# stevengiacalone/triceratops

Hardware: AMD Instinct MI355X
Metric: light-curve-point x sample evals/sec (higher is better)
Workload: dtype f64

## Files before the change

include/trx_debug.h:

```cpp
#ifndef TRX_DEBUG_H
#define TRX_DEBUG_H

#include "trx.h"

#ifdef __cplusplus
extern "C" {
#endif

int trx_set_rows_per_wave(int rows);
int trx_set_cell_packing_below(int n_time);
int trx_debug_batch_plan(long rows, int rows_per_wave, int taper, long* positions, int* rows_min);

int trx_set_supersample_tiers(int on);
int trx_set_stencil(int on);
int trx_set_skip_excluded(int on);
int trx_set_debug_node_counts(int on);
int trx_set_kepler_stepping(int on);

int trx_set_bounded_evaluation(int mode);
int trx_set_debug_bounded_lnl(int on);
int trx_set_debug_poison(int on);
int trx_set_debug_bug(int on);
int trx_set_probe_rows(int rows);
int trx_set_star_chain(int on);
int trx_debug_chain_counts(long* chains, long* calls_in_chains, long* posterior_calls_in_chains, int reset);

int trx_debug_capture_buffers(long* live, long* idle);

#ifdef __cplusplus
}
#endif
#endif
```

triceratops_amd/_lib.py:

```python
import ctypes
import os
import threading

import numpy as np
import torch

_HERE = os.path.dirname(os.path.abspath(__file__))
LIB_PATH = os.environ.get("TRX_LIB") or os.path.join(_HERE, "libtrx.so")
TESTING_LIB_PATH = os.environ.get("TRX_TESTING_LIB") or os.path.join(_HERE, "libtrx_testing.so")

MODEL_TP, MODEL_EB, MODEL_EB_TWIN, MODEL_RAW = 0, 1, 2, 3
FLAG_COMPANION_IS_HOST, FLAG_SCALAR_K, FLAG_FP32_MODEL, FLAG_EVALUATE_EXCLUDED = 1, 2, 4, 8
FLAG_ALL_SUBEXPOSURES, FLAG_NO_STENCIL, FLAG_COUNT_EVALUATIONS, FLAG_FULL_EVALUATION = 16, 32, 64, 128
FLAG_WEIGHT_MOMENTS = 256
N_PARAM = {MODEL_TP: 10, MODEL_EB: 11, MODEL_EB_TWIN: 11, MODEL_RAW: 9}
ERR_NTOTAL = 4

ABI_SYMBOLS = (
    "trx_lnl_batch", "trx_lnl_batch_weighted", "trx_flux_grid", "trx_chi2_grid", "trx_chi2_grid_weighted",
    "trx_chi2_grid_offset", "trx_chi2_grid_baseline", "trx_workspace_bytes",
    "trx_log_mean_exp", "trx_lnz_scenario", "trx_lnz_from_halfchi2", "trx_lnz_moments_from_halfchi2",
    "trx_posterior_from_halfchi2", "trx_grid_quantiles",
    "trx_lnl_batch_host", "trx_flux_grid_host",
    "trx_log_mean_exp_host", "trx_skipped_rows", "trx_pruned_rows",
    "trx_draw_scenario", "trx_draw_args_size", "trx_scenario_evidence", "trx_scenario_enqueue", "trx_star_enqueue",
    "trx_scenario_args_size", "trx_release_scratch", "trx_version", "trx_last_error", "trx_device_count",
)
DEBUG_SYMBOLS = (
    "trx_set_rows_per_wave", "trx_set_cell_packing_below", "trx_debug_batch_plan", "trx_set_supersample_tiers",
    "trx_set_stencil", "trx_set_skip_excluded", "trx_set_debug_node_counts", "trx_set_kepler_stepping",
    "trx_set_bounded_evaluation", "trx_set_debug_bounded_lnl", "trx_set_debug_poison", "trx_set_debug_bug",
    "trx_set_probe_rows", "trx_set_star_chain", "trx_debug_capture_buffers", "trx_debug_chain_counts",
)


class TrxError(RuntimeError):
    pass


EXTRA_FLAGS = 0
CELL_PACKING_BELOW = 320
STATS = {"rows": 0, "cells": 0, "launches": 0, "native_calls": 0}
_stats_lock = threading.Lock()


def count_launch(rows, n_time):
    with _stats_lock:
        STATS["rows"] += rows
        STATS["cells"] += rows * n_time
        STATS["launches"] += 1
TRACE = None
TRACE_SAMPLE_ROWS = 128


def reset_stats():
# ... 89 lines not shown
    L.trx_posterior_from_halfchi2.argtypes = [_vp, _vp, c_long, c_double, c_int, ctypes.c_ulonglong, _vp, _vp, _vp,
                                              c_size_t, _vp]
    L.trx_grid_quantiles.restype = c_int
    L.trx_grid_quantiles.argtypes = [_vp, c_long, c_int, _vp, _vp, c_long, _vp, c_int, _vp, _vp]
    L.trx_lnl_batch_host.restype = c_int
    L.trx_lnl_batch_host.argtypes = [c_int, c_int, _vp, _vp, c_int, c_double, _vp, c_long,
                                     c_double, c_int, _vp]
    L.trx_flux_grid_host.restype = c_int
    L.trx_flux_grid_host.argtypes = [c_int, c_int, _vp, c_int, _vp, c_long, c_double, c_int, _vp, _vp]
    L.trx_log_mean_exp_host.restype = c_int
    L.trx_log_mean_exp_host.argtypes = [_vp, c_long, c_long, _vp]
    L.trx_skipped_rows.restype = c_int
    L.trx_skipped_rows.argtypes = [ctypes.POINTER(ctypes.c_ulonglong), c_int]
    L.trx_pruned_rows.restype = c_int
    L.trx_pruned_rows.argtypes = [ctypes.POINTER(ctypes.c_ulonglong), c_int]
    L.trx_version.restype = ctypes.c_char_p
    L.trx_last_error.restype = ctypes.c_char_p
    L.trx_device_count.restype = c_int
    L.trx_testing = bool(testing)
    if testing:
        for name in ("trx_set_rows_per_wave", "trx_set_kepler_stepping", "trx_set_skip_excluded",
                     "trx_set_bounded_evaluation", "trx_set_debug_bounded_lnl", "trx_set_debug_poison",
                     "trx_set_debug_bug", "trx_set_star_chain", "trx_set_probe_rows", "trx_set_stencil",
                     "trx_set_supersample_tiers", "trx_set_debug_node_counts", "trx_set_cell_packing_below"):
            fn = getattr(L, name)
            fn.restype = c_int
            fn.argtypes = [c_int]
        L.trx_debug_capture_buffers.restype = c_int
        L.trx_debug_capture_buffers.argtypes = [ctypes.POINTER(c_long), ctypes.POINTER(c_long)]
    return L


def check(rc):
    if rc:
        msg = lib().trx_last_error().decode()
        if rc == ERR_NTOTAL:
            raise ValueError(msg)
        raise TrxError("libtrx error %d: %s" % (rc, msg))


def version():
    return lib().trx_version().decode()


_gpu_seen = False


def require_gpu():
    global _gpu_seen
    if _gpu_seen:
        return
    if not torch.cuda.is_available() or lib().trx_device_count() < 1:
# ... 116 lines not shown
def pack_params(model, cols, n=None):
    assert len(cols) == N_PARAM[model], (len(cols), N_PARAM[model])
    if n is None:
        n = max(int(np.size(c)) for c in cols)
    out = np.empty((len(cols), n), dtype=np.float64)
    for i, c in enumerate(cols):
        out[i] = c
    return out


def lnl_batch(model, flags, time_d, flux_d, sigma, params_d, exptime, nsamples, out=None):
    require_gpu()
    n = params_d.shape[1]
    assert params_d.shape[0] == N_PARAM[model] and params_d.is_contiguous()
    if out is None:
        out = torch.empty(n, dtype=torch.float64, device=params_d.device)
    with torch.cuda.device(params_d.device):
        check(lib().trx_lnl_batch(model, flags, time_d.data_ptr(), flux_d.data_ptr(),
                                  time_d.numel(), float(sigma), params_d.data_ptr(), n,
                                  float(exptime), int(nsamples), out.data_ptr(), _stream(params_d)))
    return out


def lnl_batch_weighted(model, flags, time_d, flux_d, inv_var_d, params_d, exptime, nsamples, sec_limit=float("inf"),
                       out=None):
    require_gpu()
    n, nt = params_d.shape[1], time_d.numel()
    assert params_d.shape[0] == N_PARAM[model] and params_d.is_contiguous()
    assert flux_d.numel() == nt and inv_var_d.numel() == nt
    assert time_d.is_contiguous() and flux_d.is_contiguous() and inv_var_d.is_contiguous()
    accumulate = out is not None
    if out is None:
        out = torch.empty(n, dtype=torch.float64, device=params_d.device)
    assert out.shape == (n,) and out.dtype == torch.float64 and out.is_contiguous()
    if n == 0:
        return out
    with torch.cuda.device(params_d.device):
        check(lib().trx_lnl_batch_weighted(model, flags, time_d.data_ptr(), flux_d.data_ptr(), inv_var_d.data_ptr(),
                                           nt, params_d.data_ptr(), n, float(exptime), int(nsamples),
                                           float(sec_limit), int(accumulate), out.data_ptr(), _stream(params_d)))
    return out


def flux_grid(model, flags, time_d, params_d, exptime, nsamples, want_secdepth=True, out=None):
    require_gpu()
    n = params_d.shape[1]
# ... 231 lines not shown
```

triceratops_amd/csrc/trx_cells.hpp:

```cpp
#pragma once
#include <hip/hip_runtime.h>
#include <math.h>

#include <cstddef>
#include <cstdint>

#include "../../include/trx.h"
#include "trx_device.hpp"
#include "trx_internal.hpp"

namespace {

using namespace trx;

constexpr int MODE_LNL = 0;
constexpr int MODE_GRID = 1;

struct RowsArgs {
    int model, flags;
    const double* time;
    const double* flux;
    int n_time;
    double sigma;
    const double* params;
// ... 22 lines not shown
    const long* n_dev;
    const int* src_idx;
    long src_stride;
    int twin_cols;
    int dense;
    int forced_B;
    int prune;
    int pstride;
    int pstride3;
    double prune_c0;
    const double* prune_lp;
    int part;
    int split;
    int* surv_list;
    unsigned long long* surv_count;
    int* probe_list;
    unsigned long long* probe_count;
    TierHead tiers;
    const double* tier_xw;
    double s2, rs2, dS, rS;
    const double* inv_var;
    double sec_limit;
    int accumulate;
};

#ifndef TRX_CHAIN_MAX_BRANCHES
#define TRX_CHAIN_MAX_BRANCHES 24
#endif
struct BranchArgs {
    int model, flags, twin_cols, need_sec;
    const double* flux;
    double sigma, s2, rs2, prune_c0;
    const double* params;
    double* out;
    const long* n_dev;
    const int* src_idx;
    const double* prune_lp;
    double* scratch;
    unsigned long long* scan_count;
};
constexpr int kChainMaxBranches = TRX_CHAIN_MAX_BRANCHES;
struct BranchTab {
    BranchArgs b[kChainMaxBranches];
};
static_assert(sizeof(RowsArgs) + sizeof(BranchTab) + 16 <= 4096, "kernel argument buffer");

// ... 18 lines not shown
    return ((w >> (i & 31)) & 1u) != 0u;
}

__device__ __forceinline__ long row_pos(const RowsArgs& a, long row)
{
    if (a.dense) return a.twin_cols ? a.src_stride - 1 - row : row;
    return a.src_idx ? (long)a.src_idx[row] : row;
}

__device__ __forceinline__ int lanes_below(unsigned long long m)
{
    return __builtin_amdgcn_mbcnt_hi((unsigned)(m >> 32), __builtin_amdgcn_mbcnt_lo((unsigned)m, 0u));
}

#ifdef TRX_PHASE_TIMERS
__device__ unsigned long long g_phase_cycles[8];
#define TRX_TICK(var) const unsigned long long var = __builtin_readcyclecounter()
#define TRX_TOCK(slot, from) tm[slot] += __builtin_readcyclecounter() - (from)
#else
#define TRX_TICK(var)
#define TRX_TOCK(slot, from)
#endif

constexpr int kStatShards = 256, kStatPad = 16;
__device__ unsigned long long g_row_stats[2][kStatShards][kStatPad];
__device__ __forceinline__ void add_row_stat(int which, unsigned count)
{
    if (count) atomicAdd(&g_row_stats[which][(blockIdx.x + 41u * blockIdx.y) & (kStatShards - 1)][0], (unsigned long long)count);
}

__device__ __forceinline__ double k_rule(double k, bool scalar_rule)
{
    if (scalar_rule) { if (fabs(k - 1.0) < 1e-6) k *= 0.999; }
    else             { if ((k - 1.0) < 1e-6) k *= 0.999; }
    return k;
}

#ifndef TRX_BATCH_WAVES
#define TRX_BATCH_WAVES 4
#endif

constexpr int kBatchWaves = TRX_BATCH_WAVES;
__host__ __device__ constexpr int cells_waves(bool long_rows) { return long_rows ? 1 : kBatchWaves; }
#ifndef TRX_TIER_LDS
#define TRX_TIER_LDS(PRUNE, LONG) true
#endif
// ... 94 lines not shown
#ifndef TRX_ST_M
#define TRX_ST_M 8
#endif
constexpr int kStM = TRX_ST_M;
constexpr int kHdrFlat = 0, kHdrStRadius = 1, kHdrStW = 2, kHdrHmin = kHdrStW + 2 * kStM + 1, kHdrXmax = kHdrHmin + 1,
              kHdrProbe = kHdrHmin + 2;
constexpr int kHdrGrid = kHdrProbe + 1, kHdrG = kHdrGrid + 64, kHdrDoubles = kHdrG + 64;
constexpr int kHdrTrip = kHdrDoubles;
__host__ __device__ inline size_t trip_sum_doubles(int n_time) { return n_time > 0 ? ((size_t)n_time + 63) / 64 : 0; }
__host__ __device__ inline double depth_grid(int i) { return pow(10.0, -5.0 + 5.0 * (double)i / 63.0); }
#ifndef TRX_PILOT_ROWS
#define TRX_PILOT_ROWS 1024
#endif
constexpr long kPilotRows = TRX_PILOT_ROWS;
#ifndef TRX_PILOT_B
#define TRX_PILOT_B 1
#endif
constexpr int kPilotB = TRX_PILOT_B;
constexpr int kProbeMinPoints = 48;
constexpr int kProbeCells = 16;
constexpr int kThirdStride = 3;
static_assert(kHdrStW + 2 * kStM + 1 <= kHdrDoubles, "launch header");

__host__ __device__ inline size_t scan_list_doubles(long n_upper) { return 2 + (size_t)(n_upper + 1) / 2; }
__host__ __device__ inline size_t launch_scratch_doubles(long n_upper, bool split, int n_time = 0)
{
    return scan_list_doubles(n_upper) * (split ? 3 : 1) + (size_t)n_upper * kRowDoubles + kHdrDoubles + trip_sum_doubles(n_time);
}
__host__ __device__ inline void set_scratch(RowsArgs& a, double* scratch)
{
    const size_t list_doubles = scan_list_doubles(a.n);
    const bool split = a.split != 0;
    a.scan_count = reinterpret_cast<unsigned long long*>(scratch);
    a.scan_list = reinterpret_cast<int*>(scratch + 2);
    a.surv_count = split ? reinterpret_cast<unsigned long long*>(scratch + list_doubles) : nullptr;
    a.surv_list = split ? reinterpret_cast<int*>(scratch + list_doubles + 2) : nullptr;
    a.probe_count = split ? reinterpret_cast<unsigned long long*>(scratch + 2 * list_doubles) : nullptr;
    a.probe_list = split ? reinterpret_cast<int*>(scratch + 2 * list_doubles + 2) : nullptr;
    a.rowc = scratch + list_doubles * (split ? 3 : 1);
}
__device__ __forceinline__ RowsArgs star_args(const RowsArgs& common, const BranchTab& bt, int part, int branch = -1)
{
    RowsArgs a = common;
    const BranchArgs& b = bt.b[branch < 0 ? (int)blockIdx.y : branch];
    a.model = b.model; a.flags = b.flags; a.twin_cols = b.twin_cols; a.need_sec = b.need_sec;
    a.flux = b.flux; a.sigma = b.sigma; a.s2 = b.s2; a.rs2 = b.rs2; a.prune_c0 = b.prune_c0;
// ... 167 lines not shown
            }
            w *= a.rS;
        }
        pmax = __shfl(pmax, 2 * kStM + 1, 64);
        double wabs = (l <= 2 * kStM) ? fabs(w) : 0.0;
#pragma unroll
        for (int o = 32; o > 0; o >>= 1) wabs += __shfl_xor(wabs, o, 64);
        ok = ok && wabs <= 3.0;
        if (l <= 2 * kStM) hdr[kHdrStW + l] = ok ? w : 0.0;
        if (l == 0) {
            double radius = 0.0;
            if (ok) {
                radius = 1.1 * 2.0 * u * ((double)kStM + pow(pmax * 1e15, 1.0 / (2.0 * kStM + 1.0)));
                if (!(radius > 0.0 && radius <= 40.0)) radius = 0.0;
            }
            hdr[kHdrStRadius] = radius;
            if (a.memo) *a.memo = (radius > 0.0) ? 2 : 1;
        }
    }
}

constexpr unsigned long long kUnwrittenBits = 0x7ff8dead0badc0deull;

template <bool SEC, bool WT = false>
__device__ __forceinline__ void rowc_body(const RowsArgs& a)
{
    __shared__ RowC rows_out[64];
    const int lane = threadIdx.x;
    const long n = a.n_dev ? *a.n_dev : a.n;
    const long nblk = (n + 63) / 64;
    if (blockIdx.x == gridDim.x - 1) {
        launch_header<WT>(a, n);
        return;
    }
    const bool quick = SEC && a.out_sec == nullptr;
    int* list = a.scan_list;
    unsigned long long* count = a.scan_count;
    for (long blk = blockIdx.x; blk < nblk; blk += gridDim.x - 1) {
        const long base = blk * 64;
        const int nb = (int)((n - base < 64) ? (n - base) : 64);
        bool open = false;
        if (lane < nb) {
            RowC c, sc;
            double ysec, fdil;
            row_constants(a, n, base + lane, c, quick, sc, ysec, fdil);
            if (quick) {
#ifndef TRX_SEC_FULL_SCAN
                const Limb L{sc.cle, sc.cld, sc.ced};
                const double ts = __dadd_rn(__dmul_rn(0.1 / 24.0, 12.0), -0.05);
                const double f = exposure_flux(sc, L, ts, 0.0, 1, 1.0, 1.0, false, a.tiers);
                const double m = (f + ysec) / (1.0 + ysec);
                const double depth = 1.0 - (m + fdil) / (1.0 + fdil);
                if (WT ? (depth >= a.sec_limit) : !(depth < 1.5 * a.sigma)) c.excl = 1.0;
                else open = true;
#else
                open = true;
#endif
            }
            const double* src = reinterpret_cast<const double*>(&c);
            double* stage = reinterpret_cast<double*>(&rows_out[lane]);
#pragma unroll
            for (int q = 0; q < kRowDoubles; ++q) stage[q] = src[q];
        }
        if (quick) {
            const unsigned long long mo = __ballot(open);
            if (mo) {
                unsigned long long at = 0;
                if (lane == 0) at = atomicAdd(count, (unsigned long long)__popcll(mo));
                at = __shfl(at, 0, 64);
                const unsigned long long slot = at + (unsigned long long)lanes_below(mo);
                if (open && slot <= (unsigned long long)a.n) list[slot] = (int)(base + lane);
            }
        }
        if (a.mark_unwritten && lane < nb) a.out[base + lane] = __longlong_as_double((long long)kUnwrittenBits);
        __syncthreads();
        {
            const double* src = reinterpret_cast<const double*>(rows_out);
            double* out = a.rowc + base * kRowDoubles;
            for (int i = lane; i < nb * kRowDoubles; i += 64) out[i] = src[i];
        }
        __syncthreads();
    }
}

template <bool SEC, bool WT = false>
__global__ __launch_bounds__(64) void rowc_kernel(RowsArgs a)
{
    rowc_body<SEC, WT>(a);
}

__global__ __launch_bounds__(64) void rowc_kernel_star(RowsArgs common, BranchTab bt)
{
    const RowsArgs a = star_args(common, bt, 0);
    if (a.need_sec) rowc_body<true>(a);
    else rowc_body<false>(a);
}

template <int E, bool WT = false>
__device__ __forceinline__ void sec_scan_body(const RowsArgs& a)
{
    __shared__ RowC srows[E];
    __shared__ double secmin[E];
    __shared__ int secnan[E];
    const int lane = threadIdx.x;
    const long n = a.n_dev ? *a.n_dev : a.n;
    const bool all_rows = a.out_sec != nullptr;
    const int* list = a.scan_list;
    const long nu = all_rows ? n : (long)*a.scan_count;
    for (long e0 = (long)blockIdx.x * E; e0 < nu; e0 += (long)gridDim.x * E) {
        const int ne = (int)((nu - e0 < E) ? (nu - e0) : E);
        long row = 0;
// ... 59 lines not shown
    double stw[(2 * kStM + 1 + 7) & ~7];
};
constexpr int kCentreNode = 1023;

__device__ __forceinline__ double fp32_model_slack(double lb, int n_probed, double rs2)
{
    return 1e-5 * sqrt(2.0 * (double)n_probed * rs2 * fmax(lb, 0.0));
}

template <int BITS>
__device__ __forceinline__ int lane_prefix(int cnt, int& total)
{
    int off = 0;
    total = 0;
#pragma unroll
    for (int b = 0; b < BITS; ++b) {
        const unsigned long long m = __ballot((cnt >> b) & 1);
        off += lanes_below(m) << b;
        total += __popcll(m) << b;
    }
    return off;
}

__device__ __forceinline__ double depth_bound(const RowC& c)
{
    const double om4 = 1.0 / (c.cle + c.cld);
    const double u2 = c.ced * om4, u1 = c.cld * om4 - 2.0 * u2;
    double imax = fmax(1.0, 1.0 - u1 - u2);
    if (u2 > 0.0 && u1 < 0.0) imax += u1 * u1 / (4.0 * u2);
    const double d = c.k * c.k * imax * (c.cle + c.cld) * c.rdil * (1.0 + 1e-12);
    return (d >= 0.0) ? d : INFINITY;
}

__device__ __forceinline__ double depth_screen(const double* hdr, double d)
{
    if (!(d < 1.0)) return 0.0;
    int i = (int)ceilf((log10f((float)fmax(d, 1e-30)) + 5.0f) * (63.0f / 5.0f));
    i = i < 0 ? 0 : (i > 63 ? 63 : i);
    if (i > 0 && hdr[kHdrGrid + i - 1] >= d) --i;
    if (hdr[kHdrGrid + i] < d) i = (i < 63) ? i + 1 : 63;
    if (hdr[kHdrGrid + i] < d) return 0.0;
    const double g = 0.5 * hdr[kHdrG + i];
    return g - fma(1e-9, g, 1e-9);
}

__device__ __forceinline__ void tighten_bounds(double* hdr, double h, double x)
// ... 48 lines not shown
#endif
struct StarKernArgs {
    RowsArgs common;
    BranchTab bt;
    int part;
};
template <typename T>
__device__ __forceinline__ const T* kernel_arguments()
{
    typedef const __attribute__((address_space(4))) T* KernArgs;
    KernArgs p = (KernArgs)__builtin_amdgcn_kernarg_segment_ptr();
    asm volatile("" : "+s"(p));
    return (const T*)p;
}

template <int MODE, bool STEP, bool FP32, bool LONG, bool ST, bool PRUNE, int ARGS = 0, bool WT = false>
__device__ __forceinline__ void cells_body(const RowsArgs& a_in, const double st_radius)
{
    constexpr int kReload = TRX_ARGS_RELOAD ? ARGS : 0;
    const RowsArgs& a = a_in;
    static_assert(!PRUNE || (MODE == MODE_LNL && !ST), "bounded evaluation: likelihood mode, no stencil");
    static_assert(!WT || (MODE == MODE_LNL && !PRUNE), "per-point weights: likelihood mode, full evaluation");
    extern __shared__ double lds_all[];
    constexpr bool kCarry = TRX_CARRY_CELLS && STEP && !LONG;
    constexpr bool kLazyTiers = TRX_LAZY_TIERS && ST && STEP && LONG && !PRUNE;
    constexpr int W = cells_waves(LONG);
    const int wave = W > 1 ? __builtin_amdgcn_readfirstlane((int)(threadIdx.x >> 6)) : 0;
    double* tier_xw = lds_all;
    double* atab = tier_xw + 2 * kTiers * kTierMaxNodes;
    double* thead = atab + kAtanRanges * kAtanCols;
    double* lds = lds_all + a.wave_off + (size_t)wave * a.wave_doubles;
    const int Bl = LONG ? 1 : a.B;
    RowC* rows = reinterpret_cast<RowC*>(lds);
    double* hacc = lds + (size_t)Bl * kRowDoubles;
    double* hmout = hacc + Bl;
    double* hrem = hmout + Bl;
    double* hlp = hrem + Bl;
    unsigned short* pdesc = reinterpret_cast<unsigned short*>(hlp + Bl);
    constexpr int kCellsWindow = cells_window(LONG);
    unsigned short* winlist = pdesc + kCellsPairs;
    CellState& cs = *reinterpret_cast<CellState*>(winlist + kCellsWindow);
    StencilState& ss = *reinterpret_cast<StencilState*>(&cs + 1);
    const double* tl = LONG ? a.time : (lds_all + a.tl_off);
    const double* fl = LONG ? a.flux : (tl + a.n_time);
    const double* wl = LONG ? a.inv_var : (fl + a.n_time);
    if (a.use_tiers) {
// ... 60 lines not shown
        else row0 = np;
        if (!LONG && (a.part == 3 || (a.part == 2 && rlist))) B = listed_pass_rows(a, row1 - row0, a.part);
        if (!LONG && a.part == 1 && a.split) B = kPilotB < Bl ? kPilotB : Bl;
        nbatch = (row1 - row0 + B - 1) / B;
    }
    const bool third_two = PRUNE && !LONG && a.part == 3 && a.pstride3 > 1;
    const int pstride = third_two ? a.pstride3 : a.pstride;
    const bool probing = PRUNE && pstride > 1 && hdr[kHdrProbe] != 0.0 &&
                         (a.part == 0 || a.part == 2 || third_two);
    if (PRUNE && a.split && a.part == 2 && !probing) return;
    const BatchPlan bp = LONG ? BatchPlan{} : batch_plan(uniform_long(row1 - row0), __builtin_amdgcn_readfirstlane(B), !PRUNE);
    const long positions = LONG ? (nbatch + 7) / 8 : bp.P;
    const long v0 = (long)(blockIdx.x & 7) + 8 * ((long)(blockIdx.x >> 3) * W + wave);
    unsigned n_skipped = 0, n_pruned = 0;
    for (long v = v0; v < 8 * positions; v += (long)gridDim.x * W) {
        RowsArgs a_again;
        if (kReload == 2) {
            const StarKernArgs* k = kernel_arguments<StarKernArgs>();
            a_again = star_args(k->common, k->bt, k->part);
        }
        const RowsArgs& a = (kReload == 1) ? *kernel_arguments<RowsArgs>() : ((kReload == 2) ? a_again : a_in);
        long base;
        int nb;
        if (LONG) {
            const long batch = (v & 7) * positions + (v >> 3);
            if ((v >> 3) >= positions || batch >= nbatch) continue;
            base = row0 + batch * B;
            nb = (int)((row1 - base < B) ? (row1 - base) : B);
        } else {
            batch_at(bp, v & 7, v >> 3, base, nb);
            base += row0;
            if (base >= row1) continue;
            if (row1 - base < nb) nb = (int)(row1 - base);
        }
        TRX_TICK(t_pro);
        TRX_CENSUS_ADD(kCenBatch, 1);
        int rowid = (int)base + lane;
        if (PRUNE && rlist) {
            if (lane < nb) rowid = rlist[base + lane];
            double* dst = reinterpret_cast<double*>(rows);
            for (int i = lane; i < nb * kRowDoubles; i += 64) {
                const int r = i / kRowDoubles, q = i - r * kRowDoubles;
                dst[i] = a.rowc[(long)rlist[base + r] * kRowDoubles + q];
            }
        } else {
            const double* src = a.rowc + base * kRowDoubles;
            double* dst = reinterpret_cast<double*>(rows);
// ... 476 lines not shown
                    for (int o = 32; o > 0; o >>= 1) {
                        hb = fmin(hb, __shfl_xor(hb, o, 64));
                        xb = fmax(xb, __shfl_xor(xb, o, 64));
                    }
                    if (lane == 0) tighten_bounds(a.rowc + n * kRowDoubles, hb, xb);
                }
            }
        }
        wave_sync();
    }
    if (PRUNE && !LONG && a.split && a.part == 2) {
        __shared__ unsigned long long wg_at;
        __syncthreads();
        const int nk = wg_nkeep < wg_valid ? wg_nkeep : wg_valid;
        if (threadIdx.x == 0 && nk > 0) wg_at = atomicAdd(a.surv_count, (unsigned long long)nk);
        __syncthreads();
        for (int i = threadIdx.x; i < nk; i += 64 * W) a.surv_list[wg_at + i] = wg_keep[i];
    }
#undef lp_row
    if (lane == 0) {
        add_row_stat(0, n_skipped);
        add_row_stat(1, n_pruned);
    }
#ifdef TRX_PHASE_TIMERS
    TRX_TOCK(7, t_all);
    if (lane == 0)
        for (int i = 0; i < 8; ++i) atomicAdd(&g_phase_cycles[i], tm[i]);
#endif
}

template <int MODE, bool STEP, bool FP32, bool LONG, bool ST, bool PRUNE = false, int ARGS = 0, bool WT = false>
__device__ __forceinline__ void cells_entry(const RowsArgs& a)
{
    if (a.need_sec && blockIdx.x == 0 && threadIdx.x == 0) *a.scan_count = 0ull;
    if (a.n_dev) {
        const long nd = *a.n_dev;
        int B = 1;
        if (!LONG) {
            B = batch_rows(nd, a.n_time, a.forced_B);
            B = B < a.B ? B : a.B;
        }
        long rows_here = nd;
        if (PRUNE && a.part) {
            const long np = nd < kPilotRows ? nd : kPilotRows;
            rows_here = a.part == 1 ? np : nd - np;
            if (!LONG && a.part == 1 && a.split) B = kPilotB < a.B ? kPilotB : a.B;
// ... 155 lines not shown
```

triceratops_amd/csrc/trx_kernels.hip:

```cpp
#include <hip/hip_runtime.h>
#include <math.h>
#include <stdio.h>
#include <stdlib.h>
#include <string.h>

#include <atomic>
#include <cstddef>
#include <cstdint>
#include <map>
#include <mutex>
#include <utility>
#include <vector>

#include "../../include/trx.h"
#include "trx_device.hpp"
#include "trx_internal.hpp"
#include "trx_knobs.hpp"

namespace {

using namespace trx;
static_assert(kTwoPiHost == kTwoPi, "lnl_c0 (trx_internal.hpp)");

thread_local char g_err[256] = "";
// ... 168 lines not shown
            if (hipHostMalloc(reinterpret_cast<void**>(&flags), kSlots * sizeof(int),
                              hipHostMallocMapped | hipHostMallocPortable) != hipSuccess) {
                (void)hipGetLastError();
                flags = nullptr;
                return nullptr;
            }
            for (int i = 0; i < kSlots; ++i) flags[i] = 0;
        }
        for (int i = 0; i < used; ++i)
            if (keys[i].time == k.time && keys[i].n_time == k.n_time && keys[i].S == k.S && keys[i].dev == k.dev &&
                keys[i].exptime == k.exptime)
                return flags + i;
        const int i = (used < kSlots) ? used++ : (next++ % kSlots);
        keys[i] = k;
        flags[i] = 0;
        return flags + i;
    }
};
StencilMemo g_stencil_memo;


thread_local const double* t_last_rowc = nullptr;
thread_local bool t_last_pruned = false;


template <int MODE, bool LONG, bool ST, bool PRUNE, bool WT>
void launch_cells_kernel(bool step, bool fp32, unsigned grid, size_t lds, hipStream_t st, const RowsArgs& a)
{
    static_assert(MODE == MODE_LNL || !(PRUNE || WT), "PRUNE and WT exist for the likelihood mode only");
    static_assert(!ST || (LONG && !PRUNE), "the stencil: one row per wave, full evaluation");
    static_assert(!(PRUNE && WT), "a weighted launch is evaluated in full");
    const dim3 g(grid), block(LONG ? 64 : 64 * kBatchWaves);
    if constexpr (!PRUNE && !WT) {
        if (!step) {
            hipLaunchKernelGGL((cells_kernel<MODE, false, false, LONG, ST, false, false>), g, block, lds, st, a);
            return;
        }
    }
    if (fp32) hipLaunchKernelGGL((cells_kernel<MODE, true, true, LONG, ST, PRUNE, WT>), g, block, lds, st, a);
    else      hipLaunchKernelGGL((cells_kernel<MODE, true, false, LONG, ST, PRUNE, WT>), g, block, lds, st, a);
}

template <int MODE>
void launch_pruned(const RowsArgs& a, hipStream_t st, bool long_rows, bool fp32, unsigned grid, size_t lds)
{
    if constexpr (MODE == MODE_LNL) {
// ... 165 lines not shown

template <int MODE, bool WT = false>
int launch_cells(const RowsArgs& a0, hipStream_t st, bool long_rows)
{
    trx::StreamLock turn(st);
    RowsArgs a = a0;
    CellsPlan P;
    if (int rc = plan_cells<MODE>(a, long_rows, P)) return rc;
    long_rows = P.long_rows;
    const bool prune = P.prune && !WT, split = P.split, fp32 = P.fp32, step = P.step;
    const size_t lds = P.lds;
    hipStreamCaptureStatus capture = hipStreamCaptureStatusNone;
    if (hipStreamIsCapturing(st, &capture) != hipSuccess) { (void)hipGetLastError(); capture = hipStreamCaptureStatusNone; }
    const bool capturing = capture == hipStreamCaptureStatusActive;
    int verdict = 0;
    if (a.use_stencil && !capturing) {
        int dev = 0;
        TRX_HIP(hipGetDevice(&dev));
        a.memo = g_stencil_memo.slot({a.time, a.n_time, a.S, dev, a.exptime});
        if (a.memo) verdict = *static_cast<volatile int*>(a.memo);
        if (verdict == 1 || verdict == 2) a.use_stencil = 2;
    }
    void* scratch = nullptr;
    const size_t scratch_bytes = launch_scratch_doubles(a.n, split, a.use_stencil ? a.n_time : 0) * sizeof(double);
#ifdef TRX_CAPTURE_GRAPH_MEM
    if (capturing) TRX_HIP(hipMallocAsync(&scratch, scratch_bytes, st));
#else
    if (capturing) TRX_HIP(trx::capture_scratch(st, scratch_bytes, &scratch));
#endif
    else TRX_HIP(trx::stream_scratch(st, 0, scratch_bytes, &scratch));
    set_scratch(a, static_cast<double*>(scratch));
    auto fail_launch = [&](hipError_t e) {
        if (!capturing) (void)hipMemsetAsync(a.scan_count, 0, sizeof(unsigned long long), st);
        return fail(TRX_ERR_HIP, "%s (hip error %ld)", hipGetErrorString(e), (long)e);
    };
    if (a.need_sec) {
        if (capturing) TRX_HIP(hipMemsetAsync(a.scan_count, 0, sizeof(unsigned long long), st));
        hipLaunchKernelGGL((rowc_kernel<true, WT>), dim3(P.grid_rowc), dim3(64), 0, st, a);
        if (a.out_sec) hipLaunchKernelGGL(sec_scan_kernel<64>, dim3(P.grid_scan), dim3(64), 0, st, a);
        else           hipLaunchKernelGGL((sec_scan_kernel<8, WT>), dim3(P.grid_scan), dim3(64), 0, st, a);
    } else {
        hipLaunchKernelGGL((rowc_kernel<false, WT>), dim3(P.grid_rowc), dim3(64), 0, st, a);
    }
    const unsigned g2 = P.grid_main;
    t_last_rowc = a.rowc;
    t_last_pruned = prune;
    if (prune) {
        RowsArgs ap = a;
        ap.part = 1;
        launch_pruned<MODE>(ap, st, long_rows, fp32, P.grid_pilot, lds);
        if (P.passes) {
            hipLaunchKernelGGL(pilot_stats_kernel, dim3(1), dim3(256), 0, st, a.out, a.n, a.n_dev, a.rowc, a.surv_count, a.pstride,
                               a.probe_count);
            if (split) hipLaunchKernelGGL(depth_screen_kernel, dim3(P.grid_screen), dim3(256), 0, st, a);
            ap.part = 2;
            const ProbePass probe = probe_pass(ap, P, 2);
            launch_pruned<MODE>(probe.a, st, long_rows, probe.fp32, g2, probe.lds);
            if (split) {
                ap.part = 3;
                launch_pruned<MODE>(ap, st, long_rows, fp32, g2, lds);
            }
        }
    } else if (long_rows) {
        if (verdict != 2) launch_cells_kernel<MODE, true, false, false, WT>(step, fp32, g2, lds, st, a);
        if (a.use_stencil && verdict != 1) launch_cells_kernel<MODE, true, true, false, WT>(step, fp32, g2, lds, st, a);
// ... 731 lines not shown
{
    g_knob_stencil = on ? 1 : 0;
    return TRX_OK;
}

int trx_set_kepler_stepping(int on)
{
    g_knob_kepler_stepping = on ? 1 : 0;
    return TRX_OK;
}

int trx_set_supersample_tiers(int on)
{
    g_knob_tiers = on ? 1 : 0;
    return TRX_OK;
}

int trx_set_debug_node_counts(int on)
{
    g_knob_debug_nodes = on ? 1 : 0;
    return TRX_OK;
}

int trx_debug_capture_buffers(long* live, long* idle)
{
    long a = 0, b = 0;
    trx::capture_scratch_stats(&a, &b);
    if (live) *live = a;
    if (idle) *idle = b;
    return TRX_OK;
}

#endif

#ifdef TRX_CENSUS
int trx_debug_census(unsigned long long* out32, int reset)
{
    TRX_HIP(hipDeviceSynchronize());
    if (out32) TRX_HIP(hipMemcpyFromSymbol(out32, HIP_SYMBOL(trx::g_census), 32 * sizeof(unsigned long long)));
    if (reset) {
        static const unsigned long long zeros[32] = {};
        TRX_HIP(hipMemcpyToSymbol(HIP_SYMBOL(trx::g_census), zeros, sizeof(zeros)));
    }
    return TRX_OK;
}
#endif

#ifdef TRX_PHASE_TIMERS
int trx_debug_phase_cycles(unsigned long long* out8)
{
    TRX_HIP(hipDeviceSynchronize());
    TRX_HIP(hipMemcpyFromSymbol(out8, HIP_SYMBOL(g_phase_cycles), 8 * sizeof(unsigned long long)));
    unsigned long long zero[8] = {0, 0, 0, 0, 0, 0, 0, 0};
    TRX_HIP(hipMemcpyToSymbol(HIP_SYMBOL(g_phase_cycles), zero, sizeof(zero)));
    return TRX_OK;
}
#endif

int trx_release_scratch(void)
{
    std::lock_guard<std::mutex> lock(trx::g_scratch_mu);
    int cur = 0;
    TRX_HIP(hipGetDevice(&cur));
    for (auto& kv : trx::g_scratch) {
        TRX_HIP(hipSetDevice(kv.first.first));
        for (int sl = 0; sl < trx::kScratchSlots; ++sl)
            if (kv.second.p[sl]) (void)(sl == 3 ? hipHostFree(kv.second.p[sl]) : hipFree(kv.second.p[sl]));
        for (int k = 0; k < trx::kStageRing; ++k) {
            if (kv.second.stage[k]) (void)hipHostFree(kv.second.stage[k]);
            if (kv.second.stage_ev[k]) (void)hipEventDestroy(kv.second.stage_ev[k]);
        }
    }
    trx::g_scratch.clear();
    TRX_HIP(hipSetDevice(cur));
    TRX_HIP(trx::capture_scratch_release_idle());
    return TRX_OK;
}
// ... 13 lines not shown
```

triceratops_amd/csrc/trx_knobs.hpp:

```cpp
#pragma once
#include <stdlib.h>

#ifdef TRX_TESTING
#include <atomic>
#endif

namespace trx {

#ifdef TRX_TESTING
inline int knob_env_int(const char* name, int dflt)
{
    const char* e = name ? getenv(name) : nullptr;
    return (e && *e) ? atoi(e) : dflt;
}
inline long env_long(const char* name, long dflt)
{
    const char* e = getenv(name);
    return (e && *e) ? atol(e) : dflt;
}
inline double env_double(const char* name, double dflt)
{
    const char* e = getenv(name);
    return (e && *e) ? atof(e) : dflt;
}
#define TRX_KNOB(name, dflt, env)                                              \
    inline std::atomic<int> g_knob_##name{knob_env_int(env, dflt)};           \
    inline int knob_##name() { return g_knob_##name.load(std::memory_order_relaxed); }
#else
constexpr long env_long(const char*, long dflt) { return dflt; }
constexpr double env_double(const char*, double dflt) { return dflt; }
#define TRX_KNOB(name, dflt, env) \
    constexpr int knob_##name() { return dflt; }
#endif

TRX_KNOB(rows_per_wave, 0, nullptr)
TRX_KNOB(probe_rows, 0, "TRX_PROBE_ROWS")
TRX_KNOB(kepler_stepping, 1, nullptr)
TRX_KNOB(tiers, 1, nullptr)
TRX_KNOB(bounded, 2, "TRX_BOUNDED")
TRX_KNOB(bounded_lnl, 0, nullptr)
TRX_KNOB(skip_excluded, 1, nullptr)
TRX_KNOB(stencil, 1, nullptr)
TRX_KNOB(debug_nodes, 0, nullptr)
TRX_KNOB(cells_below, 320, nullptr)
TRX_KNOB(debug_bug, 0, nullptr)
TRX_KNOB(poison, 0, nullptr)
TRX_KNOB(star_chain, 1, "TRX_STAR_CHAIN")

#undef TRX_KNOB

}
```

Before: 47.17 billion.

## Schedule long-row waves dearest-first using estimated in-window cell counts

Adds a per-row cost estimate (approximate count of light-curve points inside the row's transit window) computed in the row-constant kernel, which files rows into 16 cost buckets via sharded atomic lists. The main long-row kernel then maps each workgroup to one row in descending-cost order through a prefix scan over the bucket counts. The aim is to cut the launch tail, where a few expensive rows run late on an otherwise idle GPU. In exchange it adds scratch memory, a memset, atomics and a per-wave scan, and it applies only when there is one row per workgroup and the row count fits the grid. Tail-timing instrumentation and debug hooks are added as well.

After: 49.33 billion (median of 6 runs). +4.6%, better.

```diff
diff --git a/include/trx_debug.h b/include/trx_debug.h
--- a/include/trx_debug.h
+++ b/include/trx_debug.h
@@ -23,6 +23,8 @@
 int trx_set_debug_bug(int on);
 int trx_set_probe_rows(int rows);
 int trx_set_star_chain(int on);
+int trx_set_row_order(int on);
+int trx_debug_row_order(long* n_rows, long* segment_capacity, int* counts, int* lists, double* row_blocks);
 int trx_debug_chain_counts(long* chains, long* calls_in_chains, long* posterior_calls_in_chains, int reset);
 
 int trx_debug_capture_buffers(long* live, long* idle);
diff --git a/profiles/r08/ab_line.py b/profiles/r08/ab_line.py
--- /dev/null
+++ b/profiles/r08/ab_line.py
@@ -0,0 +1,9 @@
+import json, sys
+d = json.loads(sys.stdin.read().strip().splitlines()[-1])
+sh = d.get("shapes") or {}
+b = d.get("batch") or {}
+g = lambda k: (sh.get(k) or {}).get("mean_launch_ms", float("nan"))
+print("%-7s rep %s  cfg1 %.4f ms  value %.4e/s  ms_per_step %.3f | irregular %.4f ms | n100 %.4f n200 %.4f | "
+      "64-TOI step %s ms | lnZ_checksum %.15g"
+      % (sys.argv[1], sys.argv[2], d["roofline"]["mean_launch_ms"], d["value"], d["ms_per_step"], g("n2000_irregular"),
+         g("n100"), g("n200"), ("%.2f" % b["ms_per_step"]) if "ms_per_step" in b else "-", d["lnZ_checksum"]))
diff --git a/profiles/r08/tail_once.py b/profiles/r08/tail_once.py
--- /dev/null
+++ b/profiles/r08/tail_once.py
@@ -0,0 +1,47 @@
+import ctypes, os, sys
+sys.path.insert(0, os.path.dirname(os.path.dirname(os.path.dirname(os.path.abspath(__file__)))))
+import numpy as np, torch
+from triceratops_amd import _lib, synth
+
+SLOTS, TICK_US = 4096, 0.01
+n_time, n_rows = 2000, int(sys.argv[1]) if len(sys.argv) > 1 else 100000
+L = _lib.lib()
+rng = np.random.default_rng(synth.SEED)
+t_d = _lib.dev(synth.time_grid(n_time))
+curve, _ = _lib.flux_grid(0, 0, t_d, _lib.dev(synth.reference_tp_row()), synth.EXPTIME, synth.NSAMPLES, False)
+f_d = _lib.dev(synth.noisy_light_curve(rng, curve[0].cpu().numpy()))
+out = torch.empty(n_rows, dtype=torch.float64, device="cuda")
+rows = [_lib.dev(synth.family_rows(rng, fam, n_rows)) for fam in synth.FAMILIES]
+head = (ctypes.c_ulonglong * 4)()
+finish = np.zeros(n_rows, dtype=np.uint64)
+
+
+def launch(i):
+    fam = synth.FAMILIES[i]
+    flags = (_lib.FLAG_COMPANION_IS_HOST if fam[2] else 0) | _lib.FLAG_EVALUATE_EXCLUDED
+    _lib.lnl_batch(fam[1], flags, t_d, f_d, synth.SIGMA, rows[i], synth.EXPTIME, synth.NSAMPLES, out=out)
+
+
+launch(0)
+_lib.check(L.trx_debug_tail(head, None, ctypes.c_long(0)))
+results = {}
+for order in (0, 1):
+    _lib.check(L.trx_set_row_order(order))
+    keep = []
+    for i, fam in enumerate(synth.FAMILIES):
+        launch(i)
+        _lib.check(L.trx_debug_tail(head, finish.ctypes.data_as(ctypes.POINTER(ctypes.c_ulonglong)), ctypes.c_long(n_rows)))
+        first, last_start, last_finish, busy = (int(x) for x in head)
+        span, tail = last_finish - first, last_finish - last_start
+        f = finish.astype(np.int64)
+        in_tail = np.clip(f - last_start, 0, None).sum()
+        occ = in_tail / (tail * SLOTS) if tail > 0 else 1.0
+        keep.append((span * TICK_US, tail * TICK_US, occ, tail * (1.0 - occ) / span, busy / (span * SLOTS)))
+        print("order %d  %-6s span %8.1f us  tail %7.1f us  occupancy in tail %.3f  idle share of the launch %.4f  "
+              "occupancy overall %.3f" % ((order, fam[0]) + keep[-1]))
+    results[order] = np.array(keep)
+    m = results[order].mean(axis=0)
+    print("order %d  mean   span %8.1f us  tail %7.1f us  occupancy in tail %.3f  idle share of the launch %.4f  "
+          "occupancy overall %.3f" % ((order,) + tuple(m)))
+d = results[0].mean(axis=0) - results[1].mean(axis=0)
+print("as they come -> dearest first: span %+.1f us, tail %+.1f us" % (-d[0], -d[1]))
diff --git a/triceratops_amd/_lib.py b/triceratops_amd/_lib.py
--- a/triceratops_amd/_lib.py
+++ b/triceratops_amd/_lib.py
@@ -31,6 +31,7 @@
     "trx_set_stencil", "trx_set_skip_excluded", "trx_set_debug_node_counts", "trx_set_kepler_stepping",
     "trx_set_bounded_evaluation", "trx_set_debug_bounded_lnl", "trx_set_debug_poison", "trx_set_debug_bug",
     "trx_set_probe_rows", "trx_set_star_chain", "trx_debug_capture_buffers", "trx_debug_chain_counts",
+    "trx_set_row_order", "trx_debug_row_order",
 )
 
 
@@ -166,12 +167,15 @@
         for name in ("trx_set_rows_per_wave", "trx_set_kepler_stepping", "trx_set_skip_excluded",
                      "trx_set_bounded_evaluation", "trx_set_debug_bounded_lnl", "trx_set_debug_poison",
                      "trx_set_debug_bug", "trx_set_star_chain", "trx_set_probe_rows", "trx_set_stencil",
-                     "trx_set_supersample_tiers", "trx_set_debug_node_counts", "trx_set_cell_packing_below"):
+                     "trx_set_supersample_tiers", "trx_set_debug_node_counts", "trx_set_cell_packing_below",
+                     "trx_set_row_order"):
             fn = getattr(L, name)
             fn.restype = c_int
             fn.argtypes = [c_int]
         L.trx_debug_capture_buffers.restype = c_int
         L.trx_debug_capture_buffers.argtypes = [ctypes.POINTER(c_long), ctypes.POINTER(c_long)]
+        L.trx_debug_row_order.restype = c_int
+        L.trx_debug_row_order.argtypes = [ctypes.POINTER(c_long), ctypes.POINTER(c_long), _vp, _vp, _vp]
     return L
 
 
@@ -334,6 +338,20 @@
     return out
 
 
+def debug_row_order():
+    L = lib()
+    assert L.trx_testing, "debug_row_order needs use_testing_library()"
+    n, cap = ctypes.c_long(0), ctypes.c_long(0)
+    check(L.trx_debug_row_order(ctypes.byref(n), ctypes.byref(cap), None, None, None))
+    counts = np.zeros(64, dtype=np.int32)
+    lists = np.zeros(64 * cap.value, dtype=np.int32)
+    blocks = np.zeros((n.value, 19), dtype=np.float64)
+    check(L.trx_debug_row_order(ctypes.byref(n), ctypes.byref(cap), counts.ctypes.data, lists.ctypes.data,
+                                blocks.ctypes.data))
+    lists = lists.reshape(64, cap.value)
+    return counts.reshape(16, 4), [lists[s, :max(0, min(int(counts[s]), cap.value))].copy() for s in range(64)], blocks
+
+
 def lnl_batch_weighted(model, flags, time_d, flux_d, inv_var_d, params_d, exptime, nsamples, sec_limit=float("inf"),
                        out=None):
     require_gpu()
diff --git a/triceratops_amd/csrc/trx_cells.hpp b/triceratops_amd/csrc/trx_cells.hpp
--- a/triceratops_amd/csrc/trx_cells.hpp
+++ b/triceratops_amd/csrc/trx_cells.hpp
@@ -68,6 +68,7 @@
     const double* inv_var;
     double sec_limit;
     int accumulate;
+    int* order;
 };
 
 #ifndef TRX_CHAIN_MAX_BRANCHES
@@ -132,6 +133,12 @@
 #define TRX_TOCK(slot, from)
 #endif
 
+#ifdef TRX_TAIL_TIMERS
+constexpr int kTailWaves = 1 << 17;
+__device__ unsigned long long g_tail[4] = {~0ull, 0ull, 0ull, 0ull};
+__device__ unsigned long long g_tail_finish[kTailWaves];
+#endif
+
 constexpr int kStatShards = 256, kStatPad = 16;
 __device__ unsigned long long g_row_stats[2][kStatShards][kStatPad];
 __device__ __forceinline__ void add_row_stat(int which, unsigned count)
@@ -272,6 +279,21 @@
 constexpr int kThirdStride = 3;
 static_assert(kHdrStW + 2 * kStM + 1 <= kHdrDoubles, "launch header");
 
+constexpr int kOrderBuckets = 16, kOrderShards = 4, kOrderSegs = kOrderBuckets * kOrderShards;
+constexpr int kOrderStride = 16;
+static_assert(kOrderSegs == 64, "row_order_at: one segment per lane");
+__host__ __device__ inline long order_cap(long n) { return 64 * ((((n + 63) / 64) + kOrderShards - 1) / kOrderShards); }
+__host__ __device__ inline size_t order_counter_bytes() { return (size_t)kOrderSegs * kOrderStride * sizeof(int); }
+__host__ __device__ inline size_t order_doubles(long n)
+{
+    return (order_counter_bytes() + (size_t)kOrderSegs * (size_t)order_cap(n) * sizeof(int)) / sizeof(double);
+}
+__host__ __device__ inline int order_bucket(int key, int n_time)
+{
+    const int b = (int)(((long)key * kOrderBuckets) / ((long)n_time + 1));
+    return kOrderBuckets - 1 - (b < 0 ? 0 : (b > kOrderBuckets - 1 ? kOrderBuckets - 1 : b));
+}
+
 __host__ __device__ inline size_t scan_list_doubles(long n_upper) { return 2 + (size_t)(n_upper + 1) / 2; }
 __host__ __device__ inline size_t launch_scratch_doubles(long n_upper, bool split, int n_time = 0)
 {
@@ -485,7 +507,47 @@
 
 constexpr unsigned long long kUnwrittenBits = 0x7ff8dead0badc0deull;
 
-template <bool SEC, bool WT = false>
+__device__ __attribute__((noinline)) int row_cost_key(double wlo, double whi, double nmot, double t0, double tg0, double tg1,
+                                                      int n_time, bool settled)
+{
+#pragma clang fp contract(off)
+    if (settled || n_time < 1) return 0;
+    const double w = whi - wlo;
+    if (!(w >= 0.0) || !(nmot > 0.0) || !(nmot < INFINITY)) return 0;
+    if (n_time < 2 || !(tg1 > tg0) || w >= kTwoPi) return n_time;
+    const double pa = nmot * (tg0 - t0), pb = nmot * (tg1 - t0);
+    if (!(fabs(pa) < 1e15) || !(fabs(pb) < 1e15)) return 0;
+    const double xa = pa - wlo, xb = pb - wlo;
+    const double fa = floor(xa / kTwoPi), fb = floor(xb / kTwoPi);
+    const double ra = fmin(fmax(xa - kTwoPi * fa, 0.0), w), rb = fmin(fmax(xb - kTwoPi * fb, 0.0), w);
+    const double inside = (fb * w + rb) - (fa * w + ra);
+    const double step = (pb - pa) / (double)(n_time - 1);
+    double cells = inside / step;
+    if (!(cells > 0.0)) return 0;
+    cells = fmin(cells, (double)n_time);
+    return (int)(cells + 0.5);
+}
+
+__device__ __forceinline__ void order_file_rows(int* order, int bucket, long blk, long base, long n, int lane)
+{
+    int rank = 0, mine = 0;
+#pragma unroll
+    for (int b = 0; b < kOrderBuckets; ++b) {
+        const unsigned long long mb = __ballot(bucket == b);
+        if (bucket == b) rank = lanes_below(mb);
+        if (lane == b) mine = __popcll(mb);
+    }
+    const int shard = (int)(blk & (kOrderShards - 1));
+    int at = 0;
+    if (mine > 0) at = atomicAdd(&order[(lane * kOrderShards + shard) * kOrderStride], mine);
+    at = __shfl(at, bucket < 0 ? 0 : bucket, 64);
+    const long cap = order_cap(n);
+    const long slot = (long)at + rank;
+    if (bucket >= 0 && at >= 0 && slot < cap)
+        order[kOrderSegs * kOrderStride + (long)(bucket * kOrderShards + shard) * cap + slot] = (int)(base + lane);
+}
+
+template <bool SEC, bool WT = false, bool ORDER = false>
 __device__ __forceinline__ void rowc_body(const RowsArgs& a)
 {
     __shared__ RowC rows_out[64];
@@ -503,6 +565,7 @@
         const long base = blk * 64;
         const int nb = (int)((n - base < 64) ? (n - base) : 64);
         bool open = false;
+        int bucket = -1;
         if (lane < nb) {
             RowC c, sc;
             double ysec, fdil;
@@ -520,6 +583,11 @@
                 open = true;
 #endif
             }
+            if (ORDER && a.order) {
+                const bool settled = a.skip_excl && a.model == TRX_MODEL_EB && c.excl != 0.0;
+                const double tg0 = a.n_time > 0 ? a.time[0] : 0.0, tg1 = a.n_time > 0 ? a.time[a.n_time - 1] : 0.0;
+                bucket = order_bucket(row_cost_key(c.wlo, c.whi, c.nmot, c.t0, tg0, tg1, a.n_time, settled), a.n_time);
+            }
             const double* src = reinterpret_cast<const double*>(&c);
             double* stage = reinterpret_cast<double*>(&rows_out[lane]);
 #pragma unroll
@@ -535,6 +603,7 @@
                 if (open && slot <= (unsigned long long)a.n) list[slot] = (int)(base + lane);
             }
         }
+        if (ORDER && a.order) order_file_rows(a.order, bucket, blk, base, n, lane);
         if (a.mark_unwritten && lane < nb) a.out[base + lane] = __longlong_as_double((long long)kUnwrittenBits);
         __syncthreads();
         {
@@ -546,10 +615,10 @@
     }
 }
 
-template <bool SEC, bool WT = false>
+template <bool SEC, bool WT = false, bool ORDER = false>
 __global__ __launch_bounds__(64) void rowc_kernel(RowsArgs a)
 {
-    rowc_body<SEC, WT>(a);
+    rowc_body<SEC, WT, ORDER>(a);
 }
 
 __global__ __launch_bounds__(64) void rowc_kernel_star(RowsArgs common, BranchTab bt)
@@ -655,6 +724,27 @@
     return off;
 }
 
+__device__ __forceinline__ long row_order_at(const int* __restrict__ order, long v, long n, int lane)
+{
+    const int cnt = order[lane * kOrderStride];
+    int incl = cnt;
+#pragma unroll
+    for (int o = 1; o < 64; o <<= 1) {
+        const int up = __shfl_up(incl, o, 64);
+        if (lane >= o) incl += up;
+    }
+    const long first = (long)(incl - cnt);
+    const unsigned long long below = __ballot(cnt >= 0 && first <= v);
+    const int seg = __popcll(below) - 1;
+    const long total = (long)__builtin_amdgcn_readlane(incl, 63);
+    if (seg < 0 || v >= total) return -1;
+    const long at = v - (long)__builtin_amdgcn_readlane((int)first, seg);
+    const long cap = order_cap(n);
+    if (at < 0 || at >= cap) return -1;
+    const long row = (long)__builtin_amdgcn_readfirstlane(order[kOrderSegs * kOrderStride + (long)seg * cap + at]);
+    return (row >= 0 && row < n) ? row : -1;
+}
+
 __device__ __forceinline__ double depth_bound(const RowC& c)
 {
     const double om4 = 1.0 / (c.cle + c.cld);
@@ -749,6 +839,12 @@
     static_assert(!PRUNE || (MODE == MODE_LNL && !ST), "bounded evaluation: likelihood mode, no stencil");
     static_assert(!WT || (MODE == MODE_LNL && !PRUNE), "per-point weights: likelihood mode, full evaluation");
     extern __shared__ double lds_all[];
+#ifdef TRX_TAIL_TIMERS
+    const unsigned long long tail_start = LONG ? wall_clock64() : 0ull;
+#endif
+    constexpr bool kOrdered = LONG && !PRUNE && !WT && MODE == MODE_LNL;
+    int ordered_row = -2;
+    if (kOrdered && a.order) ordered_row = (int)row_order_at(a.order, (long)blockIdx.x, a.n, (int)threadIdx.x);
     constexpr bool kCarry = TRX_CARRY_CELLS && STEP && !LONG;
     constexpr bool kLazyTiers = TRX_LAZY_TIERS && ST && STEP && LONG && !PRUNE;
     constexpr int W = cells_waves(LONG);
@@ -855,7 +951,11 @@
         const RowsArgs& a = (kReload == 1) ? *kernel_arguments<RowsArgs>() : ((kReload == 2) ? a_again : a_in);
         long base;
         int nb;
-        if (LONG) {
+        if (kOrdered && ordered_row != -2) {
+            if (v != v0 || ordered_row < 0) continue;
+            base = (long)ordered_row;
+            nb = 1;
+        } else if (LONG) {
             const long batch = (v & 7) * positions + (v >> 3);
             if ((v >> 3) >= positions || batch >= nbatch) continue;
             base = row0 + batch * B;
@@ -1378,6 +1478,16 @@
         add_row_stat(0, n_skipped);
         add_row_stat(1, n_pruned);
     }
+#ifdef TRX_TAIL_TIMERS
+    if (LONG && lane == 0) {
+        const unsigned long long tail_end = wall_clock64();
+        atomicMin(&g_tail[0], tail_start);
+        atomicMax(&g_tail[1], tail_start);
+        atomicMax(&g_tail[2], tail_end);
+        atomicAdd(&g_tail[3], tail_end - tail_start);
+        if (blockIdx.y == 0 && blockIdx.x < (unsigned)kTailWaves) g_tail_finish[blockIdx.x] = tail_end;
+    }
+#endif
 #ifdef TRX_PHASE_TIMERS
     TRX_TOCK(7, t_all);
     if (lane == 0)
diff --git a/triceratops_amd/csrc/trx_kernels.hip b/triceratops_amd/csrc/trx_kernels.hip
--- a/triceratops_amd/csrc/trx_kernels.hip
+++ b/triceratops_amd/csrc/trx_kernels.hip
@@ -214,6 +214,8 @@
 
 thread_local const double* t_last_rowc = nullptr;
 thread_local bool t_last_pruned = false;
+thread_local const int* t_last_order = nullptr;
+thread_local long t_last_order_rows = 0;
 
 
 template <int MODE, bool LONG, bool ST, bool PRUNE, bool WT>
@@ -425,7 +427,10 @@
         if (verdict == 1 || verdict == 2) a.use_stencil = 2;
     }
     void* scratch = nullptr;
-    const size_t scratch_bytes = launch_scratch_doubles(a.n, split, a.use_stencil ? a.n_time : 0) * sizeof(double);
+    const size_t launch_doubles = launch_scratch_doubles(a.n, split, a.use_stencil ? a.n_time : 0);
+    const bool ordered = MODE == MODE_LNL && !WT && long_rows && !prune && !a.n_dev && a.n_time > 0 && a.n <= (1L << 20) &&
+                         (long)P.grid_main >= a.n && knob_row_order();
+    const size_t scratch_bytes = (launch_doubles + (ordered ? order_doubles(a.n) : 0)) * sizeof(double);
 #ifdef TRX_CAPTURE_GRAPH_MEM
     if (capturing) TRX_HIP(hipMallocAsync(&scratch, scratch_bytes, st));
 #else
@@ -433,17 +438,25 @@
 #endif
     else TRX_HIP(trx::stream_scratch(st, 0, scratch_bytes, &scratch));
     set_scratch(a, static_cast<double*>(scratch));
+    if (ordered) {
+        a.order = reinterpret_cast<int*>(static_cast<double*>(scratch) + launch_doubles);
+        TRX_HIP(hipMemsetAsync(a.order, 0, order_counter_bytes(), st));
+        t_last_order = a.order;
+        t_last_order_rows = a.n;
+    }
     auto fail_launch = [&](hipError_t e) {
         if (!capturing) (void)hipMemsetAsync(a.scan_count, 0, sizeof(unsigned long long), st);
         return fail(TRX_ERR_HIP, "%s (hip error %ld)", hipGetErrorString(e), (long)e);
     };
     if (a.need_sec) {
         if (capturing) TRX_HIP(hipMemsetAsync(a.scan_count, 0, sizeof(unsigned long long), st));
-        hipLaunchKernelGGL((rowc_kernel<true, WT>), dim3(P.grid_rowc), dim3(64), 0, st, a);
+        if (ordered) hipLaunchKernelGGL((rowc_kernel<true, false, true>), dim3(P.grid_rowc), dim3(64), 0, st, a);
+        else         hipLaunchKernelGGL((rowc_kernel<true, WT>), dim3(P.grid_rowc), dim3(64), 0, st, a);
         if (a.out_sec) hipLaunchKernelGGL(sec_scan_kernel<64>, dim3(P.grid_scan), dim3(64), 0, st, a);
         else           hipLaunchKernelGGL((sec_scan_kernel<8, WT>), dim3(P.grid_scan), dim3(64), 0, st, a);
     } else {
-        hipLaunchKernelGGL((rowc_kernel<false, WT>), dim3(P.grid_rowc), dim3(64), 0, st, a);
+        if (ordered) hipLaunchKernelGGL((rowc_kernel<false, false, true>), dim3(P.grid_rowc), dim3(64), 0, st, a);
+        else         hipLaunchKernelGGL((rowc_kernel<false, WT>), dim3(P.grid_rowc), dim3(64), 0, st, a);
     }
     const unsigned g2 = P.grid_main;
     t_last_rowc = a.rowc;
@@ -1221,6 +1234,32 @@
     return TRX_OK;
 }
 
+int trx_set_row_order(int on)
+{
+    g_knob_row_order = on ? 1 : 0;
+    return TRX_OK;
+}
+
+int trx_debug_row_order(long* n_rows, long* segment_capacity, int* counts, int* lists, double* row_blocks)
+{
+    if (!t_last_order || !t_last_rowc) return fail(TRX_ERR_ARG, "trx_debug_row_order: no ordered launch yet%s", "", 0);
+    const long n = t_last_order_rows, cap = order_cap(n);
+    if (n_rows) *n_rows = n;
+    if (segment_capacity) *segment_capacity = cap;
+    if (!counts && !lists && !row_blocks) return TRX_OK;
+    TRX_HIP(hipDeviceSynchronize());
+    if (counts) {
+        std::vector<int> raw((size_t)kOrderSegs * kOrderStride);
+        TRX_HIP(hipMemcpy(raw.data(), t_last_order, raw.size() * sizeof(int), hipMemcpyDeviceToHost));
+        for (int sgm = 0; sgm < kOrderSegs; ++sgm) counts[sgm] = raw[(size_t)sgm * kOrderStride];
+    }
+    if (lists)
+        TRX_HIP(hipMemcpy(lists, t_last_order + kOrderSegs * kOrderStride, (size_t)kOrderSegs * cap * sizeof(int), hipMemcpyDeviceToHost));
+    if (row_blocks)
+        TRX_HIP(hipMemcpy(row_blocks, t_last_rowc, (size_t)n * kRowDoubles * sizeof(double), hipMemcpyDeviceToHost));
+    return TRX_OK;
+}
+
 int trx_debug_capture_buffers(long* live, long* idle)
 {
     long a = 0, b = 0;
@@ -1252,6 +1291,19 @@
     TRX_HIP(hipMemcpyFromSymbol(out8, HIP_SYMBOL(g_phase_cycles), 8 * sizeof(unsigned long long)));
     unsigned long long zero[8] = {0, 0, 0, 0, 0, 0, 0, 0};
     TRX_HIP(hipMemcpyToSymbol(HIP_SYMBOL(g_phase_cycles), zero, sizeof(zero)));
+    return TRX_OK;
+}
+#endif
+
+#ifdef TRX_TAIL_TIMERS
+int trx_debug_tail(unsigned long long* out4, unsigned long long* finish, long n)
+{
+    TRX_HIP(hipDeviceSynchronize());
+    if (n < 0 || n > kTailWaves) return fail(TRX_ERR_ARG, "trx_debug_tail: n out of range%s (n=%ld)", "", n);
+    if (out4) TRX_HIP(hipMemcpyFromSymbol(out4, HIP_SYMBOL(g_tail), 4 * sizeof(unsigned long long)));
+    if (finish && n > 0) TRX_HIP(hipMemcpyFromSymbol(finish, HIP_SYMBOL(g_tail_finish), (size_t)n * sizeof(unsigned long long)));
+    const unsigned long long fresh[4] = {~0ull, 0ull, 0ull, 0ull};
+    TRX_HIP(hipMemcpyToSymbol(HIP_SYMBOL(g_tail), fresh, sizeof(fresh)));
     return TRX_OK;
 }
 #endif
diff --git a/triceratops_amd/csrc/trx_knobs.hpp b/triceratops_amd/csrc/trx_knobs.hpp
--- a/triceratops_amd/csrc/trx_knobs.hpp
+++ b/triceratops_amd/csrc/trx_knobs.hpp
@@ -46,6 +46,7 @@
 TRX_KNOB(debug_bug, 0, nullptr)
 TRX_KNOB(poison, 0, nullptr)
 TRX_KNOB(star_chain, 1, "TRX_STAR_CHAIN")
+TRX_KNOB(row_order, 1, nullptr)
 
 #undef TRX_KNOB
 
```
